# AHartmaier/pyLabFEA

Hardware: AMD Instinct MI355X
Metric: integration-point updates/sec (wall-clock per load step in ms_per_step) (higher is better)
Workload: dtype f64

## Files before the change

### include/plfx.h

```cpp
#ifndef PLFX_H
#define PLFX_H

#include <stddef.h>
#include <stdint.h>

#ifdef __cplusplus
extern "C" {
#endif

typedef struct plfx_ctx plfx_ctx;

enum {
    PLFX_ELASTIC = 0,
    PLFX_HILL6 = 1,
    PLFX_PRINC3 = 2,
    PLFX_SVC6 = 3,
    PLFX_TRESCA = 4,
    PLFX_BARLAT = 5,
    PLFX_SVC3 = 6,
    PLFX_SVC_WH = 7,
    PLFX_SVC6_COLS = 8
};

enum {
// ... 99 lines not shown
int plfx_precond_bench(plfx_ctx *ctx, int reps, double *us_per_cycle, double *us_coarse);
int plfx_solve_fallbacks(plfx_ctx *ctx, int64_t *count);
int plfx_indefinite_info(plfx_ctx *ctx, int64_t *solves, int64_t *by_minres_surrogate, int64_t *by_gmres,
                         int64_t *surrogates_built, int64_t *elements_shifted);
int plfx_set_operator(plfx_ctx *ctx, int kind);
int plfx_matvec(plfx_ctx *ctx, const double *x, double *y);
int plfx_operator_info(plfx_ctx *ctx, int *matrix_free, int *levels_matrix_free);
int plfx_reuse_info(plfx_ctx *ctx, int *assemblies, int *bc_applications, int *solves);
int plfx_predict_info(plfx_ctx *ctx, int64_t *applied, int64_t *skipped, int64_t *rejected);
int plfx_sweep_info(plfx_ctx *ctx, int64_t *sweeps, int64_t *tangents_rewritten);
int plfx_sweep_launch_info(plfx_ctx *ctx, int64_t *heavy_skipped, int64_t *heavy_recovered);
int plfx_bc_info(plfx_ctx *ctx, int64_t *rhs_rows_only, int64_t *dinv_kept, int64_t *dinv_refreshed, int64_t *du_early);
int plfx_short_info(plfx_ctx *ctx, int64_t *dinv_deferred, int64_t *dinv_formed_late, int64_t *d_kept, int64_t *spec_merged);
int plfx_snap_info(plfx_ctx *ctx, int64_t *direct_sweeps, int64_t *direct_acknowledged, int64_t *setup_formed_late, int64_t *live_restored);
int plfx_code_info(plfx_ctx *ctx, int64_t *built, int64_t *start_launches, int64_t *b_sparse_launches, int64_t *vector_launches);
int plfx_code_get(plfx_ctx *ctx, uint8_t *out);
int plfx_dead_store_info(plfx_ctx *ctx, int64_t *armed_sweeps, int64_t *tangents_rewritten_in_armed_sweeps,
                         int64_t *test_only_starts, int64_t *test_only_retries);
enum {
    PLFX_PLANE_ON = 0,
    PLFX_PLANE_NEVER_ON = 1,
    PLFX_PLANE_SWITCH = 2,
    PLFX_PLANE_SHARDED = 3,
    PLFX_PLANE_MATERIALS = 4,
    PLFX_PLANE_STATE_SET = 5,
    PLFX_PLANE_TANGENT_SET = 6
};
int plfx_plane_info(plfx_ctx *ctx, int *mode_on, int64_t *plane_sweeps, int64_t *plane_updates, int *switched_off_by);
enum {
    PLFX_MG_TAIL_NONE = 0,
// ... 134 lines not shown
```

### pylabfea_amd/_lib.py

```python
import ctypes as C
import os

import numpy as np

_HERE = os.path.dirname(os.path.abspath(__file__))
LIB_PATH = os.environ.get('PLFX_LIB', os.path.join(_HERE, 'libplfx.so'))

ELASTIC, HILL6, PRINC3, SVC6, TRESCA, BARLAT, SVC3, SVC_WH, SVC6_COLS = 0, 1, 2, 3, 4, 5, 6, 7, 8

ST_SIG, ST_EPS, ST_EPL, ST_RES_SIG, ST_RES_DEPL, ST_ELSTIFF, ST_U, ST_F, ST_DU, ST_FYN, ST_MAXSTEPS, ST_KHARD = range(12)

FIELD_NAMES = ('strain1', 'strain2', 'strain12', 'stress1', 'stress2', 'stress12', 'plastic1', 'plastic2', 'plastic12',
               'seq', 'seqJ2', 'peeq', 'etot', 'ux', 'uy')
FIELD_ID = {n: i for i, n in enumerate(FIELD_NAMES)}

T_SWEEP, T_SPMV, T_CGUPD, T_ASSEMBLE, T_VCYCLE, T_SMOOTH, T_SWEEP_HEAVY, T_COMM = range(8)


class PlfxError(RuntimeError):
    pass


class CMaterial(C.Structure):
    _fields_ = [('kind', C.c_int32), ('sdim', C.c_int32), ('CV', C.c_double * 36),
# ... 17 lines not shown
    'plfx_precond_info', 'plfx_set_operator', 'plfx_operator_info', 'plfx_gen_structured', 'plfx_reuse_info', 'plfx_timing_select', 'plfx_finish_fetch', 'plfx_sweep_info', 'plfx_matvec', 'plfx_set_bc_plan', 'plfx_apply_bc_plan',
    'plfx_set_finish_set', 'plfx_finish_step', 'plfx_scf_all', 'plfx_comm_info', 'plfx_comm_init_callback',
    'plfx_set_bc_sources',
    'plfx_load_step', 'plfx_set_strip', 'plfx_strip_info', 'plfx_allreduce_host',
    'plfx_response_batch_kh', 'plfx_fgrad_batch_wh', 'plfx_timing_sample', 'plfx_solve_fallbacks', 'plfx_comm_selftest',
    'plfx_indefinite_info', 'plfx_pattern_selftest', 'plfx_precond_bench', 'plfx_set_wh_mode', 'plfx_wh_info', 'plfx_wh_carry', 'plfx_set_mesh_structured',
    'plfx_svc_info', 'plfx_fgrad_seq_batch', 'plfx_precond_apply', 'plfx_predict_info',
    'plfx_set_response_maxit', 'plfx_sig_princ_host', 'plfx_eig3_host',
    'plfx_svc_fit_batch', 'plfx_svc_decision_batch', 'plfx_svc_fit_wide', 'plfx_hessian_batch',
    'plfx_svr_fit_batch', 'plfx_svr_predict_multi', 'plfx_set_svr_flow', 'plfx_svr_flow_info',
    'plfx_sweep_launch_info', 'plfx_element_fields', 'plfx_bc_info', 'plfx_yield_scale',
    'plfx_committee_yf', 'plfx_committee_info',
    'plfx_tex_svc_set', 'plfx_tex_svc_yf', 'plfx_tex_svc_yield_scale', 'plfx_tex_svc_info',
    'plfx_tex_svc_fgrad', 'plfx_tex_svc_full_yf', 'plfx_tex_svc_response', 'plfx_tex_svc_flow_info',
    'plfx_flow_curve', 'plfx_flow_info', 'plfx_load_path', 'plfx_load_path_info',
    'plfx_dead_store_info', 'plfx_plane_info', 'plfx_short_info', 'plfx_snap_info', 'plfx_code_info', 'plfx_code_get',
    'plfx_set_svc_cols', 'plfx_mg_info',
    'plfx_set_svc_textures', 'plfx_set_element_textures', 'plfx_response_batch_tid', 'plfx_full_yf_batch_tid',
    'plfx_svc_textures_info',
]

_lib = None


def load():
    global _lib
    if _lib is not None:
        return _lib
    if not os.path.exists(LIB_PATH):
        raise PlfxError('libplfx.so not found at %s - build it first (__graft_entry__.build()); '
                        'pylabfea_amd has no CPU fallback' % LIB_PATH)
# ... 660 lines not shown
    def short_info(self):
        a, b, r, d = C.c_int64(), C.c_int64(), C.c_int64(), C.c_int64()
        self._chk(self.lib.plfx_short_info(self.h, C.byref(a), C.byref(b), C.byref(r), C.byref(d)))
        return a.value, b.value, r.value, d.value

    def snap_info(self):
        a, b, r, d = C.c_int64(), C.c_int64(), C.c_int64(), C.c_int64()
        self._chk(self.lib.plfx_snap_info(self.h, C.byref(a), C.byref(b), C.byref(r), C.byref(d)))
        return a.value, b.value, r.value, d.value

    def code_info(self):
        a, b, r, d = C.c_int64(), C.c_int64(), C.c_int64(), C.c_int64()
        self._chk(self.lib.plfx_code_info(self.h, C.byref(a), C.byref(b), C.byref(r), C.byref(d)))
        return a.value, b.value, r.value, d.value

    def code_get(self):
        out = np.empty(self.ndof // 2, dtype=np.uint8)
        self._chk(self.lib.plfx_code_get(self.h, _dp(out)))
        return out

    def dead_store_info(self):
        a, b, r, d = C.c_int64(), C.c_int64(), C.c_int64(), C.c_int64()
        self._chk(self.lib.plfx_dead_store_info(self.h, C.byref(a), C.byref(b), C.byref(r), C.byref(d)))
        return a.value, b.value, r.value, d.value

    PLANE_OFF_REASONS = ('on', 'no state reset yet', 'switch', 'sharded', 'materials', 'state_set', 'tangent set')

    def plane_info(self):
        on, a, b, why = C.c_int(), C.c_int64(), C.c_int64(), C.c_int()
        self._chk(self.lib.plfx_plane_info(self.h, C.byref(on), C.byref(a), C.byref(b), C.byref(why)))
# ... 319 lines not shown
```

### pylabfea_amd/csrc/plfx.hip

```cpp
#define PLFX_UNIT_CONTEXT
#define PLFX_UNIT_MESH
#define PLFX_UNIT_OPERATOR
#include "plfx_host.hpp"
#include "plfx_mg.hpp"

namespace plfx {
namespace host {

typedef struct { char internal[128]; } ncclUniqueId;
typedef int (*fn_ncclGetUniqueId)(ncclUniqueId *);
typedef int (*fn_ncclCommInitRank)(ncclComm_t *, int, ncclUniqueId, int);
typedef int (*fn_ncclAllReduce)(const void *, void *, size_t, int, int, ncclComm_t, hipStream_t);
typedef int (*fn_ncclCommDestroy)(ncclComm_t);
typedef int (*fn_ncclSend)(const void *, size_t, int, int, ncclComm_t, hipStream_t);
typedef int (*fn_ncclRecv)(void *, size_t, int, int, ncclComm_t, hipStream_t);
typedef int (*fn_ncclGroup)(void);
struct Rccl {
    void *h = nullptr;
    fn_ncclGetUniqueId GetUniqueId = nullptr;
    fn_ncclCommInitRank CommInitRank = nullptr;
    fn_ncclAllReduce AllReduce = nullptr;
    fn_ncclCommDestroy CommDestroy = nullptr;
    fn_ncclSend Send = nullptr;
    fn_ncclRecv Recv = nullptr;
// ... 442 lines not shown
        dfree(L.ainv);
    }
    c->mg.clear();
    dfree(c->mg_cls);
    dfree(c->mg_dev);
    dfree(c->dtab);
    dfree(c->Mop);
    dfree(c->colr);
    c->grid_ok = false;
    c->val_valid = false;
    c->mg_tail = -1;
    c->gx = c->gy = 0;
    c->assembled = c->bc_set = false;
    c->M_dirty = true;
    c->x_is_du = false;
    c->bc_valid = c->code_ok = false;
    c->bc_idx.clear();
    c->plan.valid = false;
    dfree(c->fin_idx);
    dfree(c->fin_dev);
    c->fin_n = 0;
    dfree(c->kw);
    dfree(c->bc_rows);
    c->bc_nrows = 0;
    c->rhs_rows_ok = c->dinv_ok = c->dinv_late = false;
    c->direct_done = c->setup_owed = c->live_owed = false;
    dfree(c->tex_ids);
    c->htex_ids.clear();
    c->tex_ids_ok = false;
}

// ... 770 lines not shown
    if (const char *e10 = getenv("PLFX_DEAD_STORES")) {
        const int v = atoi(e10);
        c->dead_stores = v == 1 || v == 2;
        c->test_starts = v == 1 || v == 3;
    }
    if (!c->reuse) c->dead_stores = c->test_starts = false;
    if (const char *e11 = getenv("PLFX_PLANE_COLS")) c->plane_switch = atoi(e11) != 0;
    if (!c->reuse) c->plane_switch = false;
    if (const char *e12 = getenv("PLFX_SHORT_SOLVE")) c->short_solve = atoi(e12) & 3;
    if (!c->reuse) c->short_solve = 0;
    if (const char *e14 = getenv("PLFX_NODE_CODE")) c->node_code = atoi(e14) & 3;
    if (!(c->node_code & 1) || !c->reuse) c->node_code = 0;
    if (const char *e13 = getenv("PLFX_DIRECT_SNAP")) c->direct_snap = atoi(e13) & 3;
    if (!(c->direct_snap & 1) || !c->reuse) c->direct_snap = 0;
    if (const char *e9 = getenv("PLFX_PREDICT")) c->predict = atoi(e9) != 0;
    {
        const char *e5 = getenv("PLFX_MAILBOX");
        if (!e5 || atoi(e5)) {
            if (hipHostMalloc((void **)&c->mbox, sizeof(CgMbox), hipHostMallocMapped | hipHostMallocCoherent) == hipSuccess)
                memset(c->mbox, 0, sizeof(CgMbox));
            else
                c->mbox = nullptr;
            c->mb_cap = 1 << 16;
            if (c->mbox && hipHostMalloc((void **)&c->mb_buf, (size_t)8 * c->mb_cap,
                                         hipHostMallocMapped | hipHostMallocCoherent) != hipSuccess) {
                c->mb_buf = nullptr;
                c->mb_cap = 0;
            }
        }
    }
// ... 729 lines not shown
#undef KALLOC
    k->grid_ok = true;
    k->grid_nodes = grid_xcd(k->nnode);
    k->op = make_op(k, k->nnode, 0, nullptr, nullptr, k->gx, k->gy, k->nel_total, k->Mop);
    rc = build_hierarchy(k, k->gx, k->gy, c->hcls[0]);
    if (rc || !mg_active(k)) {
        if (!rc) rc = fail(c, PLFX_ERR_UNSUPPORTED, "the global coarse grid %d x %d has no usable hierarchy", k->gx, k->gy);
        else c->err = k->err;
        strip_free(c);
        return rc;
    }
    S.on = true;
    c->grid_nodes = MAXPART;
    c->assembled = false, c->M_dirty = true;
    c->bc_set = false;
    c->bc_valid = c->code_ok = false;
    c->rhs_rows_ok = c->dinv_ok = false;
    c->dinv_late = c->pred_d_kept = false;
    c->x_is_du = false;
    c->memo.valid = false;
    return PLFX_OK;
}

int plfx_strip_info(plfx_ctx *c, int *active, int *halo, int *coarse_level, int *coarse_levels, int64_t *halo_refreshes,
                    int64_t *coarse_gathers, int64_t *partial_allreduces, int64_t *generator_exchanges)
{
    if (!c) return PLFX_ERR_ARG;
    const auto &S = c->strip;
    if (active) *active = S.on ? 1 : 0;
    if (halo) *halo = S.W;
    if (coarse_level) *coarse_level = S.Ld;
// ... 69 lines not shown
    if (!c) return PLFX_ERR_ARG;
    if (dinv_deferred) *dinv_deferred = c->n_dinv_deferred;
    if (dinv_formed_late) *dinv_formed_late = c->n_dinv_late;
    if (d_kept) *d_kept = c->n_d_kept;
    if (spec_merged) *spec_merged = 0;
    return PLFX_OK;
}

int plfx_code_info(plfx_ctx *c, int64_t *built, int64_t *start_launches, int64_t *b_sparse_launches, int64_t *vector_launches)
{
    if (!c) return PLFX_ERR_ARG;
    if (built) *built = c->n_code_built;
    if (start_launches) *start_launches = c->n_code_start;
    if (b_sparse_launches) *b_sparse_launches = c->n_code_bsparse;
    if (vector_launches) *vector_launches = c->n_code_vector;
    return PLFX_OK;
}

int plfx_code_get(plfx_ctx *c, uint8_t *out)
{
    if (!c || !c->ncode) return c ? fail(c, PLFX_ERR_STATE, "set_mesh first") : PLFX_ERR_STATE;
    if (!out) return fail(c, PLFX_ERR_ARG, "bad argument");
    if (!c->code_ok) return fail(c, PLFX_ERR_STATE, "no node code: apply_bc first");
    HIPCHK(c, hipMemcpyAsync(out, c->ncode, (size_t)c->nnode, hipMemcpyDeviceToHost, c->stream));
    HIPCHK(c, stream_sync(c));
    return PLFX_OK;
}

int plfx_snap_info(plfx_ctx *c, int64_t *direct_sweeps, int64_t *direct_acknowledged, int64_t *setup_formed_late, int64_t *live_restored)
{
// ... 320 lines not shown
}

namespace {
int apply_bc_impl(plfx_ctx *c, int n, const int32_t *idx, const double *du_presc, const double *w, const double *fext,
                  const int32_t *seg4, const BcSegVals *segv)
{
    const size_t nd = c->ndof;
    int rc = ensure_tmp(c, std::max(n, 1));
    if (rc) return rc;
    const bool same_set = c->bc_valid && (int)c->bc_idx.size() == n &&
                          (n == 0 || memcmp(c->bc_idx.data(), idx, (size_t)4 * n) == 0);
    if (!same_set) {
        c->code_ok = false;
        c->x_is_du = false;
        c->pred_d_kept = false;
        HIPCHK(c, hipMemsetAsync(c->is_presc, 0, 8 * nd, c->stream));
        HIPCHK(c, hipMemsetAsync(c->dup, 0, 8 * nd, c->stream));
        HIPCHK(c, hipMemsetAsync(c->wv, 0, 8 * nd, c->stream));
        c->bc_idx.assign(idx, idx + n);
        if ((size_t)n > c->bc_idx_cap) {
            dfree(c->bc_idx_dev);
            if ((rc = dalloc(c, &c->bc_idx_dev, (size_t)n))) return rc;
            c->bc_idx_cap = n;
        }
        if (n > 0) {
            HIPCHK(c, hipMemcpyAsync(c->bc_idx_dev, c->bc_idx.data(), (size_t)4 * n, hipMemcpyHostToDevice, c->stream));
        }
        {
            std::vector<char> mark(c->nnode, 0);
            const int nn = c->nnode;
// ... 21 lines not shown
            for (int k = 0; k < n; k++) code[idx[k] >> 1] |= (uint8_t)(1 << (idx[k] & 1));
            HIPCHK(c, hipMemcpyAsync(c->ncode, code.data(), code.size(), hipMemcpyHostToDevice, c->stream));
            HIPCHK(c, stream_sync(c));
            c->code_ok = true;
            c->n_code_built++;
        }
        c->bc_valid = true;
        c->rhs_rows_ok = c->dinv_ok = false;
    }
    if (c->reuse && seg4 && same_set && c->bc_set && c->bc_memo && c->bc_epoch == c->op_epoch && !fext && !c->bc_memo_fext &&
        memcmp(&c->bc_last, segv, sizeof(BcSegVals)) == 0) {
        c->n_reuse_bc++;
        return PLFX_OK;
    }
    c->memo.valid = false;
    c->bc_memo = seg4 != nullptr;
    if (seg4) {
        c->bc_last = *segv;
        c->bc_epoch = c->op_epoch;
        c->bc_memo_fext = fext != nullptr;
    }
    if (n > 0 && seg4) {
        hipLaunchKernelGGL(k_scatter_bc_plan, dim3((n + BLOCK - 1) / BLOCK), dim3(BLOCK), 0, c->stream, n, c->bc_idx_dev,
                           seg4, *segv, c->dup, c->wv, c->is_presc, same_set ? 0 : 1);
        HIPCHK(c, hipGetLastError());
    } else if (n > 0) {
        if ((size_t)n > c->stage_cap) {
            HIPCHK(c, stream_sync(c));
            if (c->stage) hipHostFree(c->stage);
            c->stage = nullptr;
            HIPCHK(c, hipHostMalloc((void **)&c->stage, (size_t)32 * n));
            c->stage_cap = n;
            c->stage_busy[0] = c->stage_busy[1] = false;
        }
        const int h = c->stage_flip;
        c->stage_flip ^= 1;
        if (!c->stage_ev[h]) HIPCHK(c, hipEventCreateWithFlags(&c->stage_ev[h], hipEventDisableTiming));
        if (c->stage_busy[h]) HIPCHK(c, hipEventSynchronize(c->stage_ev[h]));
        double *st = c->stage + (size_t)h * 2 * c->stage_cap;
        memcpy(st, du_presc, (size_t)8 * n);
        memcpy(st + n, w, (size_t)8 * n);
// ... 63 lines not shown
                  const double *fext)
{
    if (!c || !c->assembled) return c ? fail(c, PLFX_ERR_STATE, "assemble first") : PLFX_ERR_STATE;
    if (n < 0 || (n > 0 && (!idx || !du_presc || !w))) return fail(c, PLFX_ERR_ARG, "bad argument");
    for (int k = 0; k < n; k++)
        if (idx[k] < 0 || idx[k] >= c->ndof) return fail(c, PLFX_ERR_ARG, "presc_idx[%d] out of range", k);
    return apply_bc_impl(c, n, idx, du_presc, w, fext, nullptr, nullptr);
}

int plfx_set_bc_plan(plfx_ctx *c, int nseg, const int32_t *seg_len, const int32_t *idx)
{
    if (!c || !c->u) return c ? fail(c, PLFX_ERR_STATE, "set_mesh first") : PLFX_ERR_STATE;
    if (nseg < 0 || (nseg > 0 && (!seg_len || !idx))) return fail(c, PLFX_ERR_ARG, "bad argument");
    auto &P = c->plan;
    P.valid = false;
    c->bc_memo = false;
    c->memo.valid = false;
    P.nseg = nseg;
    P.seg_of.clear();
    std::vector<int32_t> all;
    for (int s2 = 0, o = 0; s2 < nseg; s2++) {
        if (seg_len[s2] < 0) return fail(c, PLFX_ERR_ARG, "negative segment length");
        for (int k = 0; k < seg_len[s2]; k++, o++) {
            if (idx[o] < 0 || idx[o] >= c->ndof) return fail(c, PLFX_ERR_ARG, "plan index %d out of range", o);
            all.push_back(idx[o]);
            P.seg_of.push_back(s2);
        }
    }
    const int n = (int)all.size();
    std::vector<int32_t> order(n);
    for (int i = 0; i < n; i++) order[i] = i;
// ... 248 lines not shown
```

### pylabfea_amd/csrc/plfx_host.hpp

```cpp
#pragma once
#include "../../include/plfx.h"
#include "plfx_kernels.hpp"
#include "plfx_tex.hpp"
#include "plfx_path.hpp"

#include <dlfcn.h>
#include <algorithm>
#include <chrono>
#include <thread>
#include <cmath>
#include <cstdarg>
#include <cstdio>
#include <cstring>
#include <map>
#include <memory>
#include <mutex>
#include <string>
#include <type_traits>
#include <vector>

#define PLFX_VERSION "0.1.0-r1"

namespace plfx {
struct MgLevDev;
// ... 145 lines not shown
    int32_t *bc_idx_dev = nullptr;
    size_t bc_idx_cap = 0;
    int32_t *bc_rows = nullptr;
    int bc_nrows = 0;
    double *kw = nullptr;
    bool bc_rows_on = true;
    bool rhs_rows_ok = false, dinv_ok = false;
    long long n_rhs_rows = 0, n_dinv_kept = 0, n_dinv_refreshed = 0, n_du_early = 0;
    int short_solve = 3;
    bool dinv_late = false, pred_d_kept = false;
    long long n_dinv_deferred = 0, n_dinv_late = 0, n_d_kept = 0;
    int node_code = 1;
    uint8_t *ncode = nullptr;
    bool code_ok = false;
    long long n_code_built = 0, n_code_start = 0, n_code_bsparse = 0, n_code_vector = 0;
    int last_heavy = -1;
    long long n_heavy_skipped = 0, n_heavy_recovered = 0;
    bool x_is_du = false;
    double *pred_x = nullptr, *pred_d = nullptr;
    bool pred_valid = false;
    bool predict = true;
    bool mg_pending = false, mg_pending_same = true;
    long long n_mg_setup = 0, n_mg_setup_skipped = 0;
    bool spec_arm = false, spec_setup = false, spec_kdu = false, spec_was_clean = false;
    int direct_snap = 3;
    bool direct_done = false, setup_owed = false, live_owed = false;
    long long n_direct_sweeps = 0, n_direct_ack = 0, n_setup_late = 0, n_live_restored = 0;
    bool dead_stores = true, test_starts = true, dead_arm = false, res_partial = false;
    long long n_dead_sweeps = 0, n_dead_tangents = 0, n_test_starts = 0, n_test_retries = 0;
    bool plane_switch = true, plane_mats_ok = false, plane_cols = false;
// ... 348 lines not shown
```

### pylabfea_amd/csrc/plfx_kernels.hpp

```cpp
#pragma once
#include "plfx_device.hpp"
#include "plfx_rayroot.hpp"

namespace plfx {

constexpr int BLOCK = 256;
constexpr int MAXMAT = 16;
constexpr int MAXCLS = 16;
constexpr int MAXPART = 1024;
#ifndef PLFX_SWEEP_WAVES
#define PLFX_SWEEP_WAVES 1
#endif

struct ClassDev {
    double bxs[4], bys[4];
    double Sxx[16], Sxy[16], Syy[16];
    double kappa, vel, lx, ly;
    int32_t mat, _pad;
};

__device__ __forceinline__ double wave_sum(double v)
{
#pragma unroll
    for (int off = 32; off > 0; off >>= 1) v += __shfl_down(v, off, 64);
// ... 2541 lines not shown
    __shared__ double sh[BLOCK / 64];
    const double bb = sum_partials(part_bb, npart, sh);
    if (threadIdx.x == 0) {
        sc->thresh2 = rtol * rtol * bb;
        sc->done = 0;
        sc->iters = -1;
        sc->rr_final = -1.;
        sc->aux = 0.;
    }
}
#endif

struct CgMbox;
#ifdef PLFX_UNIT_SOLVE
__global__ void k_cg_setup_check(const double *part_bb, const double *part_rr, int npart, double rtol, CgScalars *sc, int it_done,
                                 CgMbox *mb, unsigned long long seq);
#endif

struct CgMbox {
    unsigned long long seq;
    CgScalars sc;
};

__device__ void spec_set(CgScalars *spec, int done) { spec->done = done; }

__device__ void mbox_publish(CgMbox *mb, unsigned long long seq)
{
    __threadfence_system();
    __atomic_store_n(&mb->seq, seq, __ATOMIC_RELEASE);
}

// ... 5 lines not shown
    if (!sc->done) {
        const double rr = sum_partials(part_rr, npart, sh);
        if (threadIdx.x == 0 && (rr <= sc->thresh2 || !(rr == rr))) {
            sc->done = (rr == rr) ? 1 : 2;
            sc->iters = it_done;
            sc->rr_final = rr;
        }
    }
    if (mb && threadIdx.x == 0) {
        mb->sc = *sc;
        __threadfence_system();
        __atomic_store_n(&mb->seq, seq, __ATOMIC_RELEASE);
    }
}

__global__ void k_cg_setup_check(const double *part_bb, const double *part_rr, int npart, double rtol, CgScalars *sc, int it_done,
                                 CgMbox *mb, unsigned long long seq)
{
    __shared__ double sh[BLOCK / 64];
    const double bb = sum_partials(part_bb, npart, sh);
    const double rr = sum_partials(part_rr, npart, sh);
    if (threadIdx.x == 0) {
        const double th = rtol * rtol * bb;
        sc->thresh2 = th;
        sc->aux = 0.;
        if (rr <= th || !(rr == rr)) {
            sc->done = (rr == rr) ? 1 : 2;
            sc->iters = it_done;
            sc->rr_final = rr;
        } else {
            sc->done = 0;
            sc->iters = -1;
            sc->rr_final = -1.;
        }
        if (mb) {
            mb->sc = *sc;
            __threadfence_system();
            __atomic_store_n(&mb->seq, seq, __ATOMIC_RELEASE);
        }
    }
}
#endif

#ifdef PLFX_UNIT_CONTEXT
__global__ void __launch_bounds__(BLOCK)
k_mbox_post(const double *__restrict__ src, int n, double *__restrict__ dst, CgMbox *mb, unsigned long long seq)
{
    for (int i = threadIdx.x; i < n; i += BLOCK) dst[i] = src[i];
    __threadfence_system();
    __syncthreads();
    if (threadIdx.x == 0) __atomic_store_n(&mb->seq, seq, __ATOMIC_RELEASE);
}
#endif

#ifdef PLFX_UNIT_SOLVE
// ... 128 lines not shown
            double *__restrict__ d, const CgScalars *__restrict__ sc)
{
    if (sc && sc->done) return;
    for (size_t i = blockIdx.x * (size_t)BLOCK + threadIdx.x; i < ndof; i += (size_t)gridDim.x * BLOCK)
        d[i] = (dinv[i] != 0.) ? x[i] - xprev[i] : 0.;
}

__global__ void __launch_bounds__(BLOCK)
k_pred_advance(size_t ndof, double *__restrict__ xprev, const double *__restrict__ d)
{
    for (size_t i = blockIdx.x * (size_t)BLOCK + threadIdx.x; i < ndof; i += (size_t)gridDim.x * BLOCK) xprev[i] += d[i];
}

__global__ void __launch_bounds__(BLOCK)
k_pred_dots(size_t dof_lo, size_t dof_hi , const double *__restrict__ dinv,
            const double *__restrict__ r, const double *__restrict__ kd, double *__restrict__ part, const CgScalars *__restrict__ sc,
            const uint8_t *__restrict__ code = nullptr)
{
    __shared__ double sh[BLOCK / 64];
    if (sc->done) return;
    double a0 = 0., a1 = 0.;
    for (size_t i = dof_lo + blockIdx.x * (size_t)BLOCK + threadIdx.x; i < dof_hi; i += (size_t)gridDim.x * BLOCK) {
        if (code ? ((code[i >> 1] >> (i & 1)) & 1) != 0 : dinv[i] == 0.) continue;
        const double v = kd[i];
        a0 = fma(v, r[i], a0);
        a1 = fma(v, v, a1);
    }
    const double t0 = block_sum(a0, sh);
    const double t1 = block_sum(a1, sh);
    if (threadIdx.x == 0) {
        part[blockIdx.x] = t0;
        part[(size_t)MAXPART + blockIdx.x] = t1;
    }
}

// ... 31 lines not shown
        const double ry = fy ? fma(-alpha, ki.y, ri.y) : 0.;
        a_rr = fma(rx, rx, fma(ry, ry, a_rr));
    }
    const double t = block_sum(a_rr, sh);
    if (threadIdx.x == 0) part_rr_out[blockIdx.x] = t;
}

__global__ void __launch_bounds__(BLOCK)
k_pred_commit(size_t ndof, const CgScalars *__restrict__ sc, double *__restrict__ x, const double *__restrict__ d)
{
    const double alpha = sc->aux;
    for (size_t i = blockIdx.x * (size_t)BLOCK + threadIdx.x; i < ndof; i += (size_t)gridDim.x * BLOCK) x[i] = fma(alpha, d[i], x[i]);
}

__global__ void __launch_bounds__(BLOCK)
k_pred_finish(size_t ndof, const CgScalars *__restrict__ sc, double *__restrict__ x, double *__restrict__ d,
              double *__restrict__ xprev, const double *__restrict__ dup, const double *__restrict__ is_presc, double *__restrict__ du,
              int keep_d, const uint8_t *__restrict__ code = nullptr)
{
    if (!(sc->done == 1 && sc->iters == -2)) return;
    const double alpha = sc->aux;
    for (size_t i = blockIdx.x * (size_t)BLOCK + threadIdx.x; i < ndof; i += (size_t)gridDim.x * BLOCK) {
        const double di = d[i];
        const double xi = fma(alpha, di, x[i]);
        const bool presc = code ? ((code[i >> 1] >> (i & 1)) & 1) != 0 : is_presc[i] != 0.;
        x[i] = xi;
        du[i] = presc ? dup[i] : xi;
        const double xp = xprev[i] + di;
        xprev[i] = xp;
        if (keep_d) d[i] = presc ? 0. : xi - xp;
    }
}
#endif

#ifdef PLFX_UNIT_STEP
__global__ void __launch_bounds__(BLOCK)
// ... 602 lines not shown
```

### pylabfea_amd/csrc/plfx_solve.hip

```cpp
#define PLFX_UNIT_SOLVE
#include "plfx_host.hpp"
#include "plfx_mg.hpp"

using namespace plfx;
using namespace plfx::host;

namespace plfx {
namespace host {

unsigned long long cg_check_post(plfx_ctx *c, const double *part_rr, int gn, int it_done)
{
    if (!c->mbox) {
        hipLaunchKernelGGL(k_cg_check, dim3(1), dim3(BLOCK), 0, c->stream, part_rr, gn, c->sc, it_done,
                           (CgMbox *)nullptr, 0ull);
        return 0;
    }
    const unsigned long long seq = ++c->mbox_seq;
    hipLaunchKernelGGL(k_cg_check, dim3(1), dim3(BLOCK), 0, c->stream, part_rr, gn, c->sc, it_done, c->mbox, seq);
    return seq;
}

unsigned long long cg_setup_check_post(plfx_ctx *c, const double *part_bb, const double *part_rr, int gn, double rtol)
{
    const unsigned long long seq = c->mbox ? ++c->mbox_seq : 0ull;
    hipLaunchKernelGGL(k_cg_setup_check, dim3(1), dim3(BLOCK), 0, c->stream, part_bb, part_rr, gn, rtol, c->sc, 0, c->mbox, seq);
    return seq;
}

int cg_check_wait(plfx_ctx *c, unsigned long long seq, CgScalars *hs)
{
    if (!c->mbox) {
        HIPCHK(c, hipMemcpyAsync(hs, c->sc, sizeof(*hs), hipMemcpyDeviceToHost, c->stream));
        HIPCHK(c, stream_sync(c));
        return 0;
    }
    HIPCHK(c, hipGetLastError());
    {
        const int rcw = mbox_wait(c, seq);
        if (rcw) return rcw;
    }
// ... 227 lines not shown
}

struct SolveRun {
    double *P_pq, *P_rz[2], *P_rr[2], *P_bb;
    int olo, ohi, gn, nn;
    size_t nd;
    bool multi, mg;
    CgScalars hs;
    int done, it;
    bool pred_active, pred_fused;
    bool pred_d_ready, pred_moved;
    bool pred_finished;
    bool du_early;
    bool test_only;
    bool d_kept;
};

bool wait_first_on() { static const bool on = !(getenv("PLFX_WAIT_FIRST") && atoi(getenv("PLFX_WAIT_FIRST")) == 0); return on; }

const uint8_t *node_code(plfx_ctx *c)
{
    return ((c->node_code & 1) && c->code_ok && !c->sharded && !c->strip.on && !comm_active(c) && matfree(c) && !c->op.colr) ? c->ncode : nullptr;
}
int code_b_sparse(plfx_ctx *c, const uint8_t *code) { return (code && (c->node_code & 2) && c->rhs_rows_ok) ? 1 : 0; }

bool solve_debug_on() { static const bool on = getenv("PLFX_SOLVE_DEBUG") && atoi(getenv("PLFX_SOLVE_DEBUG")) != 0; return on; }

int precondition_rz(plfx_ctx *c, double *slot, EvPair *vcycle_ev = nullptr)
{
    bool fused = false;
// ... 32 lines not shown
    if (c->strip.on && (rc = halo_refresh(c, c->x))) return rc;
    const uint8_t *code = coded ? node_code(c) : nullptr;
    hipLaunchKernelGGL(k_compose_du, dim3(grid_for(c->ndof)), dim3(BLOCK), 0, c->stream, c->ndof, c->x, c->dup, c->is_presc, c->du,
                       (const CgScalars *)nullptr, code);
    if (code) c->n_code_vector++;
    HIPCHK(c, hipGetLastError());
    return 0;
}

void remember(plfx_ctx *c, double rtol, double relres, bool valid) { c->memo = {valid, rtol, relres}; }

int solve_start(plfx_ctx *c, SolveRun &s, double rtol, int warm, int site)
{
    const size_t nd = s.nd;
    const int nn = s.nn, gn = s.gn;
    const bool x_kept = warm && c->x_is_du;
    if (!x_kept) {
        hipLaunchKernelGGL(k_x0, dim3(grid_for(nd)), dim3(BLOCK), 0, c->stream, nd, c->du, c->is_presc, warm, 1., c->x);
        c->pred_d_kept = false;
    }
    c->x_is_du = false;
    int rc = 0;
    const long long nn_global = c->strip.on ? (long long)(c->strip.gnx + 1) * (c->gy + 1) : (long long)c->nnode;
    if (c->predict && warm && !s.multi && mg_active(c) && nn_global >= 16384) {
        if (!c->pred_x && (rc = dalloc(c, &c->pred_x, nd))) return rc;
        if (!c->pred_d && (rc = dalloc(c, &c->pred_d, nd))) return rc;
        if (c->pred_valid)
            s.pred_active = true;
        else {
            HIPCHK(c, hipMemcpyAsync(c->pred_x, c->x, 8 * nd, hipMemcpyDeviceToDevice, c->stream));
            c->pred_valid = true;
// ... 37 lines not shown
        if ((rc = halo_refresh(c, c->r))) return rc;
    }
    if (!s.mg) {
        if ((rc = ensure_dinv(c))) return rc;
        hipLaunchKernelGGL(k_cg_setup, dim3(1), dim3(BLOCK), 0, c->stream, s.P_bb, gn, rtol, c->sc);
    }
    return 0;
}

int solve_first_test(plfx_ctx *c, SolveRun &s, double rtol, int site)
{
    const size_t nd = s.nd;
    const int nn = s.nn, gn = s.gn, olo = s.olo, ohi = s.ohi;
    int rc;
    bool first_passed = false, pred_first_passed = false;
    unsigned long long seq = cg_setup_check_post(c, s.P_bb, s.P_rr[1], gn, rtol);
    const bool wait_first = wait_first_on();
    if (wait_first && s.pred_active && site >= 0 && c->first_test_hint[site] && !c->strip.on) {
        const bool early = c->bc_rows_on && c->reuse && !comm_active(c);
        if (early) {
            const uint8_t *code = node_code(c);
            hipLaunchKernelGGL(k_compose_du, dim3(grid_for(nd)), dim3(BLOCK), 0, c->stream, nd, c->x, c->dup, c->is_presc, c->du,
                               (const CgScalars *)c->sc, code);
            if (code) c->n_code_vector++;
            HIPCHK(c, hipGetLastError());
        }
        if ((rc = cg_check_wait(c, seq, &s.hs))) return rc;
        s.done = s.hs.done;
        first_passed = s.done != 0;
        if (early && s.done == 1) {
            s.du_early = true;
            c->n_du_early++;
        }
        if (s.test_only && !first_passed) {
            if ((rc = ensure_dinv(c))) return rc;
            LAUNCH_OP1(k_cg_start, matfree(c), dim3(gn), c->op, nn, 1, (const double2 *)c->x, (const double2 *)c->rhs,
                       (const double2 *)c->dinv, (double2 *)c->r, (double2 *)c->z, s.P_rz[1], s.P_rr[1], s.P_bb, olo, ohi);
            HIPCHK(c, hipGetLastError());
            s.test_only = false;
            c->n_test_retries++;
        }
    }
    if (first_passed) {
        pred_first_passed = true;
    } else if (s.pred_active) {
        if (!s.pred_fused) {
            if (s.d_kept)
                c->n_d_kept++;
            else
                hipLaunchKernelGGL(k_pred_diff, dim3(grid_for(nd)), dim3(BLOCK), 0, c->stream, nd, c->x, c->pred_x, c->dinv, c->pred_d, c->sc);
            launch_spmv_plain(c, c->pred_d, c->p[0], c->sc);
        }
        const int gp = MAXPART;
        const uint8_t *code = node_code(c);
        hipLaunchKernelGGL(k_pred_dots, dim3(gp), dim3(BLOCK), 0, c->stream, (size_t)2 * olo, (size_t)2 * ohi, c->dinv, c->r, c->p[0],
                           c->part, c->sc, code);
        HIPCHK(c, hipGetLastError());
        if (c->strip.on && (rc = part_allreduce(c, c->part, (size_t)2 * MAXPART))) return rc;
        hipLaunchKernelGGL(k_pred_try, dim3(gn), dim3(BLOCK), 0, c->stream, nn, c->sc, (const double *)c->part, gp, (const double2 *)c->r,
                           (const double2 *)c->p[0], (const double2 *)c->dinv, s.P_rr[0], olo, ohi, code);
        if (code) c->n_code_vector += 2;
        HIPCHK(c, hipGetLastError());
        if (c->strip.on && (rc = part_allreduce(c, s.P_rr[0], gn))) return rc;
        seq = cg_check_post(c, s.P_rr[0], gn, -2);
        if (!c->strip.on) {
            hipLaunchKernelGGL(k_pred_finish, dim3(grid_for(nd)), dim3(BLOCK), 0, c->stream, nd, (const CgScalars *)c->sc, c->x,
                               c->pred_d, c->pred_x, (const double *)c->dup, (const double *)c->is_presc, c->du,
                               ((c->short_solve & 2) && !comm_active(c)) ? 1 : 0, code);
            if (code) c->n_code_vector++;
        }
        if ((rc = cg_check_wait(c, seq, &s.hs))) return rc;
        s.done = s.hs.done;
        if (s.done == 1 && s.hs.iters == -2) {
            c->pred_d_kept = !c->strip.on && (c->short_solve & 2) && !comm_active(c);
            if (!c->strip.on)
                s.pred_finished = true;
            else
                hipLaunchKernelGGL(k_pred_commit, dim3(grid_for(nd)), dim3(BLOCK), 0, c->stream, nd, (const CgScalars *)c->sc, c->x, c->pred_d);
            HIPCHK(c, hipGetLastError());
            s.hs.iters = 0;
            c->n_pred++;
            s.pred_d_ready = true;
            s.pred_moved = true;
        } else if (!s.done) {
// ... 307 lines not shown
```

Measured before the change: 6.256 billion.

## Fold CG convergence tests into neighbouring kernels and skip redundant BC scatters

Three folds, all on by default through fold_tests=7. The setup-check kernel can now write prescribed rows of du directly, replacing a full-vector k_compose_du launch. In the fused-predictor path, the initial convergence test moves into k_pred_dots and the post-predictor test and mailbox publish move into k_pred_finish, which removes separate single-block check launches. The BC plan scatter is skipped when the segment values and index set match the last applied ones. This cuts kernel launches and serial single-block kernels per solve, at the cost of every pred_dots block redundantly reducing the partials and more complex mailbox/state logic.

```diff
diff --git a/include/plfx.h b/include/plfx.h
--- a/include/plfx.h
+++ b/include/plfx.h
@@ -137,6 +137,7 @@
 int plfx_short_info(plfx_ctx *ctx, int64_t *dinv_deferred, int64_t *dinv_formed_late, int64_t *d_kept, int64_t *spec_merged);
 int plfx_snap_info(plfx_ctx *ctx, int64_t *direct_sweeps, int64_t *direct_acknowledged, int64_t *setup_formed_late, int64_t *live_restored);
 int plfx_code_info(plfx_ctx *ctx, int64_t *built, int64_t *start_launches, int64_t *b_sparse_launches, int64_t *vector_launches);
+int plfx_fold_info(plfx_ctx *ctx, int64_t *rows_composed, int64_t *pred_folded, int64_t *scatters_skipped);
 int plfx_code_get(plfx_ctx *ctx, uint8_t *out);
 int plfx_dead_store_info(plfx_ctx *ctx, int64_t *armed_sweeps, int64_t *tangents_rewritten_in_armed_sweeps,
                          int64_t *test_only_starts, int64_t *test_only_retries);
diff --git a/pylabfea_amd/_lib.py b/pylabfea_amd/_lib.py
--- a/pylabfea_amd/_lib.py
+++ b/pylabfea_amd/_lib.py
@@ -55,7 +55,7 @@
     'plfx_tex_svc_set', 'plfx_tex_svc_yf', 'plfx_tex_svc_yield_scale', 'plfx_tex_svc_info',
     'plfx_tex_svc_fgrad', 'plfx_tex_svc_full_yf', 'plfx_tex_svc_response', 'plfx_tex_svc_flow_info',
     'plfx_flow_curve', 'plfx_flow_info', 'plfx_load_path', 'plfx_load_path_info',
-    'plfx_dead_store_info', 'plfx_plane_info', 'plfx_short_info', 'plfx_snap_info', 'plfx_code_info', 'plfx_code_get',
+    'plfx_dead_store_info', 'plfx_plane_info', 'plfx_short_info', 'plfx_snap_info', 'plfx_code_info', 'plfx_code_get', 'plfx_fold_info',
     'plfx_set_svc_cols', 'plfx_mg_info',
     'plfx_set_svc_textures', 'plfx_set_element_textures', 'plfx_response_batch_tid', 'plfx_full_yf_batch_tid',
     'plfx_svc_textures_info',
@@ -746,6 +746,11 @@
         self._chk(self.lib.plfx_code_info(self.h, C.byref(a), C.byref(b), C.byref(r), C.byref(d)))
         return a.value, b.value, r.value, d.value
 
+    def fold_info(self):
+        a, b, r = C.c_int64(), C.c_int64(), C.c_int64()
+        self._chk(self.lib.plfx_fold_info(self.h, C.byref(a), C.byref(b), C.byref(r)))
+        return a.value, b.value, r.value
+
     def code_get(self):
         out = np.empty(self.ndof // 2, dtype=np.uint8)
         self._chk(self.lib.plfx_code_get(self.h, _dp(out)))
diff --git a/pylabfea_amd/csrc/plfx.hip b/pylabfea_amd/csrc/plfx.hip
--- a/pylabfea_amd/csrc/plfx.hip
+++ b/pylabfea_amd/csrc/plfx.hip
@@ -480,7 +480,7 @@
     c->assembled = c->bc_set = false;
     c->M_dirty = true;
     c->x_is_du = false;
-    c->bc_valid = c->code_ok = false;
+    c->bc_valid = c->code_ok = c->bc_scatter_ok = false;
     c->bc_idx.clear();
     c->plan.valid = false;
     dfree(c->fin_idx);
@@ -1281,6 +1281,8 @@
     if (const char *e13 = getenv("PLFX_DIRECT_SNAP")) c->direct_snap = atoi(e13) & 3;
     if (!(c->direct_snap & 1) || !c->reuse) c->direct_snap = 0;
     if (const char *e9 = getenv("PLFX_PREDICT")) c->predict = atoi(e9) != 0;
+    if (const char *e15 = getenv("PLFX_FOLD_TESTS")) c->fold_tests = atoi(e15) & 7;
+    if (!c->reuse) c->fold_tests = 0;
     {
         const char *e5 = getenv("PLFX_MAILBOX");
         if (!e5 || atoi(e5)) {
@@ -2040,7 +2042,7 @@
     c->grid_nodes = MAXPART;
     c->assembled = false, c->M_dirty = true;
     c->bc_set = false;
-    c->bc_valid = c->code_ok = false;
+    c->bc_valid = c->code_ok = c->bc_scatter_ok = false;
     c->rhs_rows_ok = c->dinv_ok = false;
     c->dinv_late = c->pred_d_kept = false;
     c->x_is_du = false;
@@ -2140,6 +2142,15 @@
     if (start_launches) *start_launches = c->n_code_start;
     if (b_sparse_launches) *b_sparse_launches = c->n_code_bsparse;
     if (vector_launches) *vector_launches = c->n_code_vector;
+    return PLFX_OK;
+}
+
+int plfx_fold_info(plfx_ctx *c, int64_t *rows_composed, int64_t *pred_folded, int64_t *scatters_skipped)
+{
+    if (!c) return PLFX_ERR_ARG;
+    if (rows_composed) *rows_composed = c->n_fold_rows;
+    if (pred_folded) *pred_folded = c->n_fold_pred;
+    if (scatters_skipped) *scatters_skipped = c->n_fold_scatter;
     return PLFX_OK;
 }
 
@@ -2490,6 +2501,7 @@
         c->code_ok = false;
         c->x_is_du = false;
         c->pred_d_kept = false;
+        c->bc_scatter_ok = false;
         HIPCHK(c, hipMemsetAsync(c->is_presc, 0, 8 * nd, c->stream));
         HIPCHK(c, hipMemsetAsync(c->dup, 0, 8 * nd, c->stream));
         HIPCHK(c, hipMemsetAsync(c->wv, 0, 8 * nd, c->stream));
@@ -2541,17 +2553,23 @@
         return PLFX_OK;
     }
     c->memo.valid = false;
+    const bool scatter_stands = (c->fold_tests & 4) && n > 0 && seg4 && same_set && c->bc_memo && c->bc_scatter_ok && !c->strip.on &&
+                                !comm_active(c) && memcmp(&c->bc_last, segv, sizeof(BcSegVals)) == 0;
     c->bc_memo = seg4 != nullptr;
     if (seg4) {
         c->bc_last = *segv;
         c->bc_epoch = c->op_epoch;
         c->bc_memo_fext = fext != nullptr;
     }
-    if (n > 0 && seg4) {
+    if (scatter_stands)
+        c->n_fold_scatter++;
+    else if (n > 0 && seg4) {
         hipLaunchKernelGGL(k_scatter_bc_plan, dim3((n + BLOCK - 1) / BLOCK), dim3(BLOCK), 0, c->stream, n, c->bc_idx_dev,
                            seg4, *segv, c->dup, c->wv, c->is_presc, same_set ? 0 : 1);
         HIPCHK(c, hipGetLastError());
+        c->bc_scatter_ok = true;
     } else if (n > 0) {
+        c->bc_scatter_ok = false;
         if ((size_t)n > c->stage_cap) {
             HIPCHK(c, stream_sync(c));
             if (c->stage) hipHostFree(c->stage);
@@ -2645,7 +2663,7 @@
     if (nseg < 0 || (nseg > 0 && (!seg_len || !idx))) return fail(c, PLFX_ERR_ARG, "bad argument");
     auto &P = c->plan;
     P.valid = false;
-    c->bc_memo = false;
+    c->bc_memo = c->bc_scatter_ok = false;
     c->memo.valid = false;
     P.nseg = nseg;
     P.seg_of.clear();
diff --git a/pylabfea_amd/csrc/plfx_host.hpp b/pylabfea_amd/csrc/plfx_host.hpp
--- a/pylabfea_amd/csrc/plfx_host.hpp
+++ b/pylabfea_amd/csrc/plfx_host.hpp
@@ -183,6 +183,9 @@
     uint8_t *ncode = nullptr;
     bool code_ok = false;
     long long n_code_built = 0, n_code_start = 0, n_code_bsparse = 0, n_code_vector = 0;
+    int fold_tests = 7;
+    bool bc_scatter_ok = false;
+    long long n_fold_rows = 0, n_fold_pred = 0, n_fold_scatter = 0;
     int last_heavy = -1;
     long long n_heavy_skipped = 0, n_heavy_recovered = 0;
     bool x_is_du = false;
diff --git a/pylabfea_amd/csrc/plfx_kernels.hpp b/pylabfea_amd/csrc/plfx_kernels.hpp
--- a/pylabfea_amd/csrc/plfx_kernels.hpp
+++ b/pylabfea_amd/csrc/plfx_kernels.hpp
@@ -2579,7 +2579,8 @@
 struct CgMbox;
 #ifdef PLFX_UNIT_SOLVE
 __global__ void k_cg_setup_check(const double *part_bb, const double *part_rr, int npart, double rtol, CgScalars *sc, int it_done,
-                                 CgMbox *mb, unsigned long long seq);
+                                 CgMbox *mb, unsigned long long seq, const int32_t *idx = nullptr, int n = 0,
+                                 const double *dup = nullptr, double *du = nullptr);
 #endif
 
 struct CgMbox {
@@ -2615,14 +2616,26 @@
     }
 }
 
+constexpr int SETUP_ROWS = 8;
 __global__ void k_cg_setup_check(const double *part_bb, const double *part_rr, int npart, double rtol, CgScalars *sc, int it_done,
-                                 CgMbox *mb, unsigned long long seq)
+                                 CgMbox *mb, unsigned long long seq, const int32_t *idx, int n, const double *dup, double *du)
 {
     __shared__ double sh[BLOCK / 64];
+    int pi[SETUP_ROWS];
+    double pv[SETUP_ROWS];
+    if (idx) {
+#pragma unroll
+        for (int q = 0; q < SETUP_ROWS; q++) {
+            const int k = threadIdx.x + q * BLOCK;
+            pi[q] = k < n ? idx[k] : -1;
+        }
+#pragma unroll
+        for (int q = 0; q < SETUP_ROWS; q++) pv[q] = pi[q] >= 0 ? dup[pi[q]] : 0.;
+    }
     const double bb = sum_partials(part_bb, npart, sh);
     const double rr = sum_partials(part_rr, npart, sh);
+    const double th = rtol * rtol * bb;
     if (threadIdx.x == 0) {
-        const double th = rtol * rtol * bb;
         sc->thresh2 = th;
         sc->aux = 0.;
         if (rr <= th || !(rr == rr)) {
@@ -2640,6 +2653,23 @@
             __atomic_store_n(&mb->seq, seq, __ATOMIC_RELEASE);
         }
     }
+    if (idx && rr <= th) {
+#pragma unroll
+        for (int q = 0; q < SETUP_ROWS; q++)
+            if (pi[q] >= 0) du[pi[q]] = pv[q];
+        for (int base = SETUP_ROWS * BLOCK; base < n; base += SETUP_ROWS * BLOCK) {
+#pragma unroll
+            for (int q = 0; q < SETUP_ROWS; q++) {
+                const int k = base + threadIdx.x + q * BLOCK;
+                pi[q] = k < n ? idx[k] : -1;
+            }
+#pragma unroll
+            for (int q = 0; q < SETUP_ROWS; q++) pv[q] = pi[q] >= 0 ? dup[pi[q]] : 0.;
+#pragma unroll
+            for (int q = 0; q < SETUP_ROWS; q++)
+                if (pi[q] >= 0) du[pi[q]] = pv[q];
+        }
+    }
 }
 #endif
 
@@ -2798,11 +2828,34 @@
 
 __global__ void __launch_bounds__(BLOCK)
 k_pred_dots(size_t dof_lo, size_t dof_hi , const double *__restrict__ dinv,
-            const double *__restrict__ r, const double *__restrict__ kd, double *__restrict__ part, const CgScalars *__restrict__ sc,
-            const uint8_t *__restrict__ code = nullptr)
+            const double *__restrict__ r, const double *__restrict__ kd, double *__restrict__ part, CgScalars *sc,
+            const uint8_t *__restrict__ code = nullptr, const double *part_bb = nullptr, const double *part_rr = nullptr, int npart = 0,
+            double rtol = 0.)
 {
     __shared__ double sh[BLOCK / 64];
-    if (sc->done) return;
+    if (part_bb) {
+        const double *const two[2] = {part_bb, part_rr};
+        double o[2];
+        sum_partials_n<2>(two, npart, o);
+        const double bb = o[0], rr = o[1];
+        const double th = rtol * rtol * bb;
+        const bool passed = rr <= th || !(rr == rr);
+        if (blockIdx.x == 0 && threadIdx.x == 0) {
+            sc->thresh2 = th;
+            sc->aux = 0.;
+            if (passed) {
+                sc->done = (rr == rr) ? 1 : 2;
+                sc->iters = 0;
+                sc->rr_final = rr;
+            } else {
+                sc->done = 0;
+                sc->iters = -1;
+                sc->rr_final = -1.;
+            }
+        }
+        if (passed) return;
+    } else if (sc->done)
+        return;
     double a0 = 0., a1 = 0.;
     for (size_t i = dof_lo + blockIdx.x * (size_t)BLOCK + threadIdx.x; i < dof_hi; i += (size_t)gridDim.x * BLOCK) {
         if (code ? ((code[i >> 1] >> (i & 1)) & 1) != 0 : dinv[i] == 0.) continue;
@@ -2864,12 +2917,28 @@
 }
 
 __global__ void __launch_bounds__(BLOCK)
-k_pred_finish(size_t ndof, const CgScalars *__restrict__ sc, double *__restrict__ x, double *__restrict__ d,
+k_pred_finish(size_t ndof, CgScalars *sc, double *__restrict__ x, double *__restrict__ d,
               double *__restrict__ xprev, const double *__restrict__ dup, const double *__restrict__ is_presc, double *__restrict__ du,
-              int keep_d, const uint8_t *__restrict__ code = nullptr)
-{
-    if (!(sc->done == 1 && sc->iters == -2)) return;
+              int keep_d, const uint8_t *__restrict__ code = nullptr, const double *part_rr = nullptr, int npart = 0,
+              CgMbox *mb = nullptr, unsigned long long seq = 0ull)
+{
     const double alpha = sc->aux;
+    if (part_rr) {
+        __shared__ double sh[BLOCK / 64];
+        const double th = sc->thresh2;
+        const double rr = sum_partials(part_rr, npart, sh);
+        if (blockIdx.x == 0 && threadIdx.x == 0) {
+            if (!sc->done && (rr <= th || !(rr == rr))) {
+                sc->done = (rr == rr) ? 1 : 2;
+                sc->iters = -2;
+                sc->rr_final = rr;
+            }
+            mb->sc = *sc;
+            mbox_publish(mb, seq);
+        }
+        if (!(alpha != 0. && rr <= th)) return;
+    } else if (!(sc->done == 1 && sc->iters == -2))
+        return;
     for (size_t i = blockIdx.x * (size_t)BLOCK + threadIdx.x; i < ndof; i += (size_t)gridDim.x * BLOCK) {
         const double di = d[i];
         const double xi = fma(alpha, di, x[i]);
diff --git a/pylabfea_amd/csrc/plfx_solve.hip b/pylabfea_amd/csrc/plfx_solve.hip
--- a/pylabfea_amd/csrc/plfx_solve.hip
+++ b/pylabfea_amd/csrc/plfx_solve.hip
@@ -20,10 +20,11 @@
     return seq;
 }
 
-unsigned long long cg_setup_check_post(plfx_ctx *c, const double *part_bb, const double *part_rr, int gn, double rtol)
+unsigned long long cg_setup_check_post(plfx_ctx *c, const double *part_bb, const double *part_rr, int gn, double rtol, bool rows = false)
 {
     const unsigned long long seq = c->mbox ? ++c->mbox_seq : 0ull;
-    hipLaunchKernelGGL(k_cg_setup_check, dim3(1), dim3(BLOCK), 0, c->stream, part_bb, part_rr, gn, rtol, c->sc, 0, c->mbox, seq);
+    hipLaunchKernelGGL(k_cg_setup_check, dim3(1), dim3(BLOCK), 0, c->stream, part_bb, part_rr, gn, rtol, c->sc, 0, c->mbox, seq,
+                       rows ? (const int32_t *)c->bc_idx_dev : nullptr, rows ? (int)c->bc_idx.size() : 0, (const double *)c->dup, c->du);
     return seq;
 }
 
@@ -281,6 +282,7 @@
     bool du_early;
     bool test_only;
     bool d_kept;
+    bool x_kept;
 };
 
 bool wait_first_on() { static const bool on = !(getenv("PLFX_WAIT_FIRST") && atoi(getenv("PLFX_WAIT_FIRST")) == 0); return on; }
@@ -343,7 +345,7 @@
 {
     const size_t nd = s.nd;
     const int nn = s.nn, gn = s.gn;
-    const bool x_kept = warm && c->x_is_du;
+    const bool x_kept = s.x_kept = warm && c->x_is_du;
     if (!x_kept) {
         hipLaunchKernelGGL(k_x0, dim3(grid_for(nd)), dim3(BLOCK), 0, c->stream, nd, c->du, c->is_presc, warm, 1., c->x);
         c->pred_d_kept = false;
@@ -411,11 +413,15 @@
     const int nn = s.nn, gn = s.gn, olo = s.olo, ohi = s.ohi;
     int rc;
     bool first_passed = false, pred_first_passed = false;
-    unsigned long long seq = cg_setup_check_post(c, s.P_bb, s.P_rr[1], gn, rtol);
     const bool wait_first = wait_first_on();
-    if (wait_first && s.pred_active && site >= 0 && c->first_test_hint[site] && !c->strip.on) {
-        const bool early = c->bc_rows_on && c->reuse && !comm_active(c);
-        if (early) {
+    const bool wait_here = wait_first && s.pred_active && site >= 0 && c->first_test_hint[site] && !c->strip.on;
+    const bool early = wait_here && c->bc_rows_on && c->reuse && !comm_active(c);
+    const bool early_rows = early && (c->fold_tests & 1) && s.x_kept && c->bc_idx_dev && c->bc_idx.size() <= (size_t)64 * BLOCK;
+    const bool fold_pred = (c->fold_tests & 2) && s.pred_fused && !wait_here && c->mbox && !c->strip.on && !comm_active(c);
+    unsigned long long seq = 0ull;
+    if (!fold_pred) seq = cg_setup_check_post(c, s.P_bb, s.P_rr[1], gn, rtol, early_rows);
+    if (wait_here) {
+        if (early && !early_rows) {
             const uint8_t *code = node_code(c);
             hipLaunchKernelGGL(k_compose_du, dim3(grid_for(nd)), dim3(BLOCK), 0, c->stream, nd, c->x, c->dup, c->is_presc, c->du,
                                (const CgScalars *)c->sc, code);
@@ -428,6 +434,7 @@
         if (early && s.done == 1) {
             s.du_early = true;
             c->n_du_early++;
+            if (early_rows) c->n_fold_rows++;
         }
         if (s.test_only && !first_passed) {
             if ((rc = ensure_dinv(c))) return rc;
@@ -450,8 +457,12 @@
         }
         const int gp = MAXPART;
         const uint8_t *code = node_code(c);
-        hipLaunchKernelGGL(k_pred_dots, dim3(gp), dim3(BLOCK), 0, c->stream, (size_t)2 * olo, (size_t)2 * ohi, c->dinv, c->r, c->p[0],
-                           c->part, c->sc, code);
+        if (fold_pred)
+            hipLaunchKernelGGL(k_pred_dots, dim3(gp), dim3(BLOCK), 0, c->stream, (size_t)2 * olo, (size_t)2 * ohi, c->dinv, c->r, c->p[0],
+                               c->part, c->sc, code, (const double *)s.P_bb, (const double *)s.P_rr[1], gn, rtol);
+        else
+            hipLaunchKernelGGL(k_pred_dots, dim3(gp), dim3(BLOCK), 0, c->stream, (size_t)2 * olo, (size_t)2 * ohi, c->dinv, c->r, c->p[0],
+                               c->part, c->sc, code);
         HIPCHK(c, hipGetLastError());
         if (c->strip.on && (rc = part_allreduce(c, c->part, (size_t)2 * MAXPART))) return rc;
         hipLaunchKernelGGL(k_pred_try, dim3(gn), dim3(BLOCK), 0, c->stream, nn, c->sc, (const double *)c->part, gp, (const double2 *)c->r,
@@ -459,12 +470,21 @@
         if (code) c->n_code_vector += 2;
         HIPCHK(c, hipGetLastError());
         if (c->strip.on && (rc = part_allreduce(c, s.P_rr[0], gn))) return rc;
-        seq = cg_check_post(c, s.P_rr[0], gn, -2);
-        if (!c->strip.on) {
-            hipLaunchKernelGGL(k_pred_finish, dim3(grid_for(nd)), dim3(BLOCK), 0, c->stream, nd, (const CgScalars *)c->sc, c->x,
-                               c->pred_d, c->pred_x, (const double *)c->dup, (const double *)c->is_presc, c->du,
-                               ((c->short_solve & 2) && !comm_active(c)) ? 1 : 0, code);
+        if (fold_pred) {
+            seq = ++c->mbox_seq;
+            hipLaunchKernelGGL(k_pred_finish, dim3(grid_for(nd)), dim3(BLOCK), 0, c->stream, nd, c->sc, c->x, c->pred_d, c->pred_x,
+                               (const double *)c->dup, (const double *)c->is_presc, c->du, (c->short_solve & 2) ? 1 : 0, code,
+                               (const double *)s.P_rr[0], gn, c->mbox, seq);
             if (code) c->n_code_vector++;
+            c->n_fold_pred++;
+        } else {
+            seq = cg_check_post(c, s.P_rr[0], gn, -2);
+            if (!c->strip.on) {
+                hipLaunchKernelGGL(k_pred_finish, dim3(grid_for(nd)), dim3(BLOCK), 0, c->stream, nd, c->sc, c->x,
+                                   c->pred_d, c->pred_x, (const double *)c->dup, (const double *)c->is_presc, c->du,
+                                   ((c->short_solve & 2) && !comm_active(c)) ? 1 : 0, code);
+                if (code) c->n_code_vector++;
+            }
         }
         if ((rc = cg_check_wait(c, seq, &s.hs))) return rc;
         s.done = s.hs.done;
```

After: 6.259 billion, median of 2. No clear change (+0.0%).
